# rhymes-ai/Aria

Measured on NVIDIA H100. Metric: Aria-25.3B bf16 prefill tokens/sec, higher is better.
Workload: dtype bf16

## Files before the change

aria_b200/csrc/gemm.cu:

```cuda
#include "gemm_common.cuh"

namespace aria {

constexpr int GEMM_STAGES = 4;
constexpr int acc_ld(int BN) { return BN + 4; }
template <int BN>
constexpr int gemm_smem_bytes() {
  return 1024  + GEMM_STAGES * (A_STAGE_BYTES + BN * BK * 2) + BM * acc_ld(BN) * 4 + 256 ;
}

template <int BN, bool B_MN>
ARIA_DEVICE void wgmma_tile_k16(float (&acc)[BN / 2], uint64_t da, uint64_t db) {
  if constexpr (BN == 128) wgmma_m64n128_ss<0, B_MN ? 1 : 0>(acc, da, db, 1u);
  else wgmma_m64n144_ss<0, B_MN ? 1 : 0>(acc, da, db, 1u);
}

template <int BN, bool B_MN, int EPI>
__global__ void __launch_bounds__(GEMM_THREADS, 1)
gemm_kernel(const __grid_constant__ CUtensorMap tmA, const __grid_constant__ CUtensorMap tmB0,
            const __grid_constant__ CUtensorMap tmB1, const __grid_constant__ CUtensorMap tmB2, const GemmParams p) {
  constexpr int B_STAGE_BYTES = BN * BK * 2;
  constexpr int STAGE_BYTES = A_STAGE_BYTES + B_STAGE_BYTES;
  constexpr int STAGES = GEMM_STAGES;
  constexpr int ACC_LD = acc_ld(BN);
  constexpr int OUT_BN = (EPI == ARIA_EPI_SWIGLU) ? BN / 2 : BN;
  static_assert(BN == 128 || BN == 144, "tile widths with a wgmma wrapper");

  extern __shared__ uint8_t smem_raw[];
  uint8_t* smem = reinterpret_cast<uint8_t*>((reinterpret_cast<uintptr_t>(smem_raw) + 1023) & ~uintptr_t(1023));
  float* stg = reinterpret_cast<float*>(smem + STAGES * STAGE_BYTES);
  uint64_t* full_bar = reinterpret_cast<uint64_t*>(stg + BM * ACC_LD);
  uint64_t* empty_bar = full_bar + STAGES;

  const int warp = threadIdx.x >> 5;
  const int lane = threadIdx.x & 31;
  const int wg = threadIdx.x >> 7;

  if (warp == 0 && lane == 0) {
    prefetch_tmap(&tmA);
    prefetch_tmap(&tmB0);
    if (p.n_seg > 1 || EPI == ARIA_EPI_SWIGLU) prefetch_tmap(&tmB1);
    if (p.n_seg > 2) prefetch_tmap(&tmB2);
    for (int i = 0; i < STAGES; ++i) {
      mbar_init(&full_bar[i], 1);
      mbar_init(&empty_bar[i], CONSUMER_WARPS);
    }
    fence_mbar_init();
  }
  __syncthreads();

  const int n_out_total = p.N * (EPI == ARIA_EPI_SWIGLU ? 1 : p.n_seg);
  const int n_tiles = (n_out_total + OUT_BN - 1) / OUT_BN;
  const int k_blocks = (p.K + BK - 1) / BK;
  const uint32_t smem_base = smem_u32(smem);
  const uint32_t full0 = smem_u32(full_bar), empty0 = smem_u32(empty_bar);

  if (wg == 0) {
    setmaxnreg_dec<40>();
    if (warp == 0 && elect_one()) {
      TileSched sched;
      sched.init(p, n_tiles);
      uint32_t stage = 0, phase = 0;
      for (int t = blockIdx.x;; t += gridDim.x) {
        int grp, m_idx, n_idx, row0, rows;
        if (!sched.decode(t, grp, m_idx, n_idx, row0, rows)) break;
        const int a_row = row0 + m_idx * BM;
        const int bgrp = weight_block(p, grp);
        int b_c0 = 0, b_c1 = 0;
        const CUtensorMap* tb0 = &tmB0;
        const CUtensorMap* tb1 = &tmB1;
        if constexpr (B_MN) {
          b_c0 = bgrp * p.K;
        } else if constexpr (EPI == ARIA_EPI_SWIGLU) {
          b_c0 = b_c1 = n_idx * OUT_BN;
        } else {
          const int col = n_idx * BN;
          const int seg = col / p.N;
          tb0 = seg == 0 ? &tmB0 : (seg == 1 ? &tmB1 : &tmB2);
          b_c0 = col - seg * p.N + bgrp * p.b_group_rows;
        }
        for (int kb = 0; kb < k_blocks; ++kb) {
          const uint32_t fb = full0 + stage * 8;
          const uint32_t sa = smem_base + stage * STAGE_BYTES;
          const uint32_t sb = sa + A_STAGE_BYTES;
          mbar_wait_addr(empty0 + stage * 8, phase ^ 1);
          mbar_arrive_expect_tx_addr(fb, STAGE_BYTES);
          tma_load_2d_addr(sa, &tmA, fb, kb * BK, a_row);
          if constexpr (B_MN) {
            const int krow = b_c0 + kb * BK;
            constexpr int CH = BN / 64;
#pragma unroll
            for (int c = 0; c < CH; ++c) {
              int ncol;
              if constexpr (EPI == ARIA_EPI_SWIGLU) {
                constexpr int HALF = CH / 2;
                ncol = (c < HALF) ? (n_idx * OUT_BN + c * 64) : (p.N + n_idx * OUT_BN + (c - HALF) * 64);
              } else {
                ncol = n_idx * BN + c * 64;
              }
              tma_load_2d_addr(sb + c * (64 * BK * 2), &tmB0, fb, ncol, krow);
            }
          } else if constexpr (EPI == ARIA_EPI_SWIGLU) {
            tma_load_2d_addr(sb, tb0, fb, kb * BK, b_c0);
            tma_load_2d_addr(sb + (BN / 2) * BK * 2, tb1, fb, kb * BK, b_c1);
          } else {
            tma_load_2d_addr(sb, tb0, fb, kb * BK, b_c0);
          }
          if (++stage == STAGES) {
            stage = 0;
            phase ^= 1;
          }
        }
      }
    }
  } else {
    setmaxnreg_inc<232>();
    const int cw = wg - 1;
    const int tid = threadIdx.x & 127;
    const uint32_t b_lbo = p.dbg_lbo ? p.dbg_lbo : (B_MN ? 64 * BK * 2 : 16);
    const uint32_t b_sbo = p.dbg_sbo ? p.dbg_sbo : 1024;
    const uint32_t b_kadv = (p.dbg_kadv ? p.dbg_kadv : (B_MN ? 16 * 128 : 32)) >> 4;
    const uint64_t da0 = make_smem_desc(smem_base + cw * 64 * 128, 16, 1024);
    const uint64_t db0 = make_smem_desc(smem_base + A_STAGE_BYTES, b_lbo, b_sbo);
    const int frag_row = cw * 64 + (tid >> 5) * 16 + (lane >> 2), frag_col = 2 * (lane & 3);
    const int epi_row = cw * 64 + (tid & 63), half = tid >> 6;
    TileSched sched;
    sched.init(p, n_tiles);
    uint32_t stage = 0, phase = 0;
    for (int t = blockIdx.x;; t += gridDim.x) {
      int grp, m_idx, n_idx, row0, rows;
      if (!sched.decode(t, grp, m_idx, n_idx, row0, rows)) break;
      float acc[BN / 2];
#pragma unroll
      for (int i = 0; i < BN / 2; ++i) acc[i] = 0.f;
      int prev = -1;
      for (int kb = 0; kb < k_blocks; ++kb) {
        mbar_wait_addr(full0 + stage * 8, phase);
        const uint64_t da = da0 + stage * (STAGE_BYTES >> 4);
        const uint64_t db = db0 + stage * (STAGE_BYTES >> 4);
        wgmma_fence();
#pragma unroll
        for (int k = 0; k < BK / 16; ++k) wgmma_tile_k16<BN, B_MN>(acc, da + k * 2, db + k * b_kadv);
        wgmma_commit();
        wgmma_wait<1>();
        if (prev >= 0 && lane == 0) mbar_arrive(&empty_bar[prev]);
        prev = static_cast<int>(stage);
        if (++stage == STAGES) {
          stage = 0;
          phase ^= 1;
        }
      }
      wgmma_wait<0>();
      fence_regs(acc);
      if (prev >= 0 && lane == 0) mbar_arrive(&empty_bar[prev]);

      named_bar_sync(1 + cw, 128);
#pragma unroll
      for (int j = 0; j < BN / 8; ++j) {
        float* d0 = stg + frag_row * ACC_LD + 8 * j + frag_col;
        *reinterpret_cast<float2*>(d0) = make_float2(acc[4 * j], acc[4 * j + 1]);
        *reinterpret_cast<float2*>(d0 + 8 * ACC_LD) = make_float2(acc[4 * j + 2], acc[4 * j + 3]);
      }
      named_bar_sync(1 + cw, 128);
      const int r_in_grp = m_idx * BM + epi_row;
      const bool row_ok = r_in_grp < rows;
      const int64_t grow = static_cast<int64_t>(row0) + r_in_grp;
      epilogue_tile<BN, EPI>(p, stg + epi_row * ACC_LD, n_out_total, n_idx, grow, row_ok, half, grp, r_in_grp);
    }
  }
}

template <int BN, bool B_MN, int EPI>
static int launch_gemm(const CUtensorMap& tmA, const CUtensorMap* tmB, const GemmParams& p, int max_tiles,
                       cudaStream_t stream) {
  constexpr int SMEM = gemm_smem_bytes<BN>();
  auto kern = gemm_kernel<BN, B_MN, EPI>;
  static bool attr_set[kMaxDevices] = {};
  if (ensure_dynamic_smem(attr_set, kern, SMEM) != cudaSuccess) return ARIA_ERR_CUDA;
  int grid = sm_count();
  if (max_tiles < grid) grid = max_tiles;
  if (grid < 1) grid = 1;
  kern<<<grid, GEMM_THREADS, SMEM, stream>>>(tmA, tmB[0], tmB[1], tmB[2], p);
  return check_launch("gemm_kernel");
}

}

using namespace aria;

extern "C" int aria_gemm(const aria_gemm_desc_t* d, aria_stream_t stream_) {
  cudaStream_t stream = reinterpret_cast<cudaStream_t>(stream_);
  ARIA_CHECK_ARG(d != nullptr);
  ARIA_CHECK_ARG(d->a && d->b[0] && d->out[0]);
  ARIA_CHECK_ARG(d->m >= 0 && d->n > 0 && d->k > 0);
  ARIA_CHECK_ARG(d->n % 8 == 0 && d->k % 8 == 0 && d->lda % 8 == 0);
  ARIA_CHECK_ARG(d->n_seg >= 1 && d->n_seg <= 3);
  ARIA_CHECK_ARG(d->num_groups >= 1 && (d->group_mod >= 0 || d->num_groups % (-d->group_mod) == 0));
  ARIA_CHECK_ARG((reinterpret_cast<uintptr_t>(d->a) & 15) == 0 && (reinterpret_cast<uintptr_t>(d->out[0]) & 15) == 0);
  if (d->m == 0) return ARIA_OK;
  const bool b_mn = d->b_layout == ARIA_B_GKN;
  const bool b_gnk = d->b_layout == ARIA_B_GNK;
  const bool swiglu = d->epilogue == ARIA_EPI_SWIGLU;
  if (b_mn) {
    ARIA_CHECK_ARG(d->n_seg == 1);
    ARIA_CHECK_ARG(d->k % BK == 0 || (d->num_groups == 1 && d->group_mod == 0));
    ARIA_CHECK_ARG(d->n % 64 == 0);
// ... 23 lines not shown
  p.n_seg = swiglu ? 1 : d->n_seg;
  p.act = d->act;
  for (int i = 0; i < 3; ++i) {
    p.bias[i] = static_cast<const __nv_bfloat16*>(d->bias[i]);
    p.out[i] = static_cast<__nv_bfloat16*>(d->out[i]);
  }
  p.residual = static_cast<const __nv_bfloat16*>(d->residual);
  p.ldr = d->ldr;
  p.ldo = d->ldo;
  p.head_dim = d->head_dim;
  p.head_ld = d->head_ld;
  p.rows_per_batch = d->rows_per_batch > 0 ? d->rows_per_batch : static_cast<int>(d->m);
  p.pos0 = d->pos0;
  p.stride_b = d->stride_b;
  p.stride_h = d->stride_h;
  p.rope_mask = d->rope_mask;
  p.rope_cos = static_cast<const __nv_bfloat16*>(d->rope_cos);
  p.rope_sin = static_cast<const __nv_bfloat16*>(d->rope_sin);
  p.position_ids = d->position_ids;
  p.dbg_lbo = d->dbg_lbo;
  p.dbg_sbo = d->dbg_sbo;
  p.dbg_kadv = d->dbg_kadv;

  const int64_t n_out_total = d->n * (swiglu ? 1 : d->n_seg);
  int BN = 128;
  if (d->epilogue == ARIA_EPI_HEADS) {
    ARIA_CHECK_ARG(d->head_dim > 0 && d->head_dim % 8 == 0 && d->head_ld >= d->head_dim && d->n % d->head_dim == 0);
    if (d->rope_mask) ARIA_CHECK_ARG(d->head_dim == 128 && d->rope_cos && d->rope_sin);
    if (d->n % 128 != 0) {
      ARIA_CHECK_ARG(!d->rope_mask && d->n % 144 == 0);
      BN = 144;
    }
    for (int s = 0; s < d->n_seg; ++s) ARIA_CHECK_ARG(d->out[s] && d->b[s]);
  } else {
    if (swiglu) ARIA_CHECK_ARG(d->n % 64 == 0);
    if (d->n_seg > 1 && !swiglu) ARIA_CHECK_ARG(d->n % BN == 0);
  }

  CUtensorMap tmA, tmB[3];
  int rc = make_tmap_2d(&tmA, d->a, d->k, d->a_rows > 0 ? d->a_rows : d->m, d->lda * 2, BK, BM);
  if (rc) return rc;
  if (b_mn) {
    const uint64_t ncols = swiglu ? 2 * d->n : d->n;
    const uint64_t n_weights = d->group_mod > 0 ? d->group_mod : (d->group_mod < 0 ? d->num_groups / (-d->group_mod) : d->num_groups);
    rc = make_tmap_2d(&tmB[0], d->b[0], ncols, n_weights * d->k, ncols * 2, 64, BK);
    if (rc) return rc;
    tmB[1] = tmB[0];
    tmB[2] = tmB[0];
  } else {
    const int nb = swiglu ? 2 : d->n_seg;
    const uint32_t box_rows = swiglu ? BN / 2 : BN;
    for (int s = 0; s < 3; ++s) {
      const void* ptr = s < nb ? d->b[s] : d->b[0];
      const uint64_t b_rows = b_gnk ? static_cast<uint64_t>(d->group_mod > 0 ? d->group_mod : (d->group_mod < 0 ? d->num_groups / (-d->group_mod) : d->num_groups)) * d->n : d->n;
      rc = make_tmap_2d(&tmB[s], ptr, d->k, b_rows, d->k * 2, BK, box_rows);
      if (rc) return rc;
    }
  }

  const int out_bn = swiglu ? BN / 2 : BN;
  const int64_t n_tiles = (n_out_total + out_bn - 1) / out_bn;
  const int64_t m_tiles_ub = (d->m + BM - 1) / BM + (d->num_groups > 1 ? d->num_groups : 0);
  int64_t max_tiles = n_tiles * m_tiles_ub;
  if (max_tiles > (1 << 30)) max_tiles = 1 << 30;

#define ARIA_LAUNCH(BN_, MN_, EPI_) return launch_gemm<BN_, MN_, EPI_>(tmA, tmB, p, static_cast<int>(max_tiles), stream)
  if (d->epilogue == ARIA_EPI_HEADS) {
    if (BN == 128) ARIA_LAUNCH(128, false, ARIA_EPI_HEADS);
    ARIA_LAUNCH(144, false, ARIA_EPI_HEADS);
  }
  if (swiglu) {
    if (b_mn) ARIA_LAUNCH(128, true, ARIA_EPI_SWIGLU);
    ARIA_LAUNCH(128, false, ARIA_EPI_SWIGLU);
  }
  if (b_mn) ARIA_LAUNCH(128, true, ARIA_EPI_LINEAR);
  ARIA_LAUNCH(128, false, ARIA_EPI_LINEAR);
#undef ARIA_LAUNCH
}

extern "C" int aria_grouped_gemm(const void* a, const void* b, void* out, const int32_t* group_offsets, int64_t rows,
                                 int64_t k, int64_t n, int32_t num_groups, aria_stream_t stream) {
  aria_gemm_desc_t d{};
  d.a = a;
  d.lda = k;
  d.m = rows;
  d.n = n;
  d.k = k;
  d.b[0] = b;
  d.n_seg = 1;
  d.b_layout = ARIA_B_GKN;
  d.num_groups = num_groups;
  d.group_offsets = group_offsets;
  d.epilogue = ARIA_EPI_LINEAR;
// ... 8 lines not shown
```

aria_b200/csrc/gemm_common.cuh:

```cuda
#pragma once
#include "common.cuh"
#include "ptx.cuh"

namespace aria {

constexpr int BM = 128;
constexpr int BK = 64;
constexpr int A_STAGE_BYTES = BM * BK * 2;
constexpr int GEMM_THREADS = 384;
constexpr int CONSUMER_WARPS = 8;

struct GemmParams {
  int M, N, K;
  int num_groups;
  const int32_t* group_offsets;
  const int32_t* group_counts;
  const uint64_t* out_group_base;
  const int32_t* out_group_row0;
  int b_group_rows;
  int group_mod;
  int n_seg;
  int act;
  const __nv_bfloat16* bias[3];
  const __nv_bfloat16* residual;
// ... 28 lines not shown
    g = -1;
    mt_prefix = 0;
    g_mt = 0;
    g_row0 = 0;
    g_rows = 0;
  }
  __device__ bool load_group(int gi) {
    if (gi >= G) return false;
    if (offs) {
      g_row0 = offs[gi];
      g_rows = cnts ? cnts[gi] : offs[gi + 1] - g_row0;
    } else {
      g_row0 = 0;
      g_rows = M;
    }
    g_mt = (g_rows + bm - 1) / bm;
    return true;
  }
  __device__ bool decode(int t, int& grp, int& m_idx, int& n_idx, int& row0, int& rows) {
    if (g < 0) {
      g = 0;
      if (!load_group(0)) return false;
    }
    while (t >= (mt_prefix + g_mt) * n_tiles) {
      mt_prefix += g_mt;
      ++g;
      if (!load_group(g)) return false;
    }
    int r = t - mt_prefix * n_tiles;
    n_idx = r / g_mt;
    m_idx = r - n_idx * g_mt;
    grp = g;
    row0 = g_row0;
    rows = g_rows;
    return true;
  }
};

ARIA_DEVICE float act_apply(float x, int act) {
  if (act == ARIA_ACT_GELU_TANH) {
    const float k0 = 0.7978845608028654f, k1 = 0.044715f;
    float inner = k0 * (x + k1 * x * x * x);
    return 0.5f * x * (1.f + fast_tanh(inner));
  }
  if (act == ARIA_ACT_GELU_NEW) {
    float p3 = bf16r(x * x * x);
    float t = bf16r(0.044715f * p3);
    t = bf16r(x + t);
    t = bf16r(0.7978845608028654f * t);
    t = bf16r(fast_tanh(t));
    t = bf16r(1.0f + t);
    float h = bf16r(0.5f * x);
    return h * t;
  }
  return x;
}

ARIA_DEVICE void ld_acc32(const float* src, uint32_t (&r)[32]) {
#pragma unroll
  for (int i = 0; i < 8; ++i) {
    const uint4 v = *reinterpret_cast<const uint4*>(src + 4 * i);
    r[4 * i] = v.x;
    r[4 * i + 1] = v.y;
    r[4 * i + 2] = v.z;
    r[4 * i + 3] = v.w;
  }
}

template <int BN, int EPI>
ARIA_DEVICE void epilogue_tile(const GemmParams& p, const float* acc, const int n_out_total, const int n_idx,
                               const int64_t grow, const bool row_ok, const int half, const int grp = 0, const int r_in_grp = 0) {
  constexpr int OUT_BN = (EPI == ARIA_EPI_SWIGLU) ? BN / 2 : BN;
  if constexpr (EPI == ARIA_EPI_SWIGLU) {
    __nv_bfloat16* orow = p.out[0] + grow * p.ldo + n_idx * OUT_BN;
    constexpr int NCH = OUT_BN / 32;
    const int cb = (half * NCH / 2) * 32, ce = half ? OUT_BN : (NCH / 2) * 32;
#pragma unroll 1
    for (int c = cb; c < ce; c += 32) {
      uint32_t g[32], u[32];
      ld_acc32(acc + c, g);
      ld_acc32(acc + OUT_BN + c, u);
      uint32_t o[16];
#pragma unroll
      for (int j = 0; j < 32; j += 2) {
        float g0 = __uint_as_float(g[j]), g1 = __uint_as_float(g[j + 1]);
        float u0 = __uint_as_float(u[j]), u1 = __uint_as_float(u[j + 1]);
        bf16r2(g0, g1);
        bf16r2(u0, u1);
        float s0 = fast_silu(g0), s1 = fast_silu(g1);
        bf16r2(s0, s1);
        o[j >> 1] = pack_bf16(s0 * u0, s1 * u1);
      }
      if (row_ok) {
#pragma unroll
        for (int q = 0; q < 4; ++q) {
          const int col = n_idx * OUT_BN + c + q * 8;
          if (col + 8 <= p.N)
            *reinterpret_cast<uint4*>(orow + c + q * 8) = make_uint4(o[q * 4], o[q * 4 + 1], o[q * 4 + 2], o[q * 4 + 3]);
        }
      }
    }
  } else if constexpr (EPI == ARIA_EPI_LINEAR) {
    const int col0 = n_idx * BN;
    const int seg = col0 / p.N;
    const __nv_bfloat16* bias = p.bias[seg];
    __nv_bfloat16* orow = p.out[0] + grow * p.ldo + col0;
    if (p.out_group_base)
      orow = reinterpret_cast<__nv_bfloat16*>(p.out_group_base[grp]) + static_cast<int64_t>(p.out_group_row0[grp] + r_in_grp) * p.ldo + col0;
    const __nv_bfloat16* rrow = (p.residual && row_ok) ? p.residual + grow * p.ldr + col0 : nullptr;
    constexpr int NCH = BN / 32, NCHH = NCH - NCH / 2;
    const int cb = half ? (NCH / 2) * 32 : 0;
    const int n_my = half ? NCH - NCH / 2 : NCH / 2;
    if (n_my == 0) return;
    uint32_t v[2][32];
    uint4 bv[2][4], rv[2][4];
    auto issue = [&](int c, int set) {
      ld_acc32(acc + c, v[set]);
#pragma unroll
      for (int q = 0; q < 4; ++q) {
        const int col = col0 + c + q * 8;
        const bool ok = col + 8 <= n_out_total;
        bv[set][q] = (bias && ok) ? __ldg(reinterpret_cast<const uint4*>(bias + (col - seg * p.N))) : make_uint4(0, 0, 0, 0);
        rv[set][q] = (rrow && ok) ? *reinterpret_cast<const uint4*>(rrow + c + q * 8) : make_uint4(0, 0, 0, 0);
      }
    };
    issue(cb, 0);
#pragma unroll
    for (int i = 0; i < NCHH; ++i) {
      if (i >= n_my) break;
      const int c = cb + i * 32;
      const int set = i & 1;
      if (i + 1 < n_my) issue(c + 32, set ^ 1);
#pragma unroll
      for (int q = 0; q < 4; ++q) {
        const int col = col0 + c + q * 8;
        if (col + 8 > n_out_total) continue;
        float x[8];
#pragma unroll
        for (int j = 0; j < 8; ++j) x[j] = __uint_as_float(v[set][q * 8 + j]);
        if (bias) {
          const uint32_t bw[4] = {bv[set][q].x, bv[set][q].y, bv[set][q].z, bv[set][q].w};
#pragma unroll
          for (int j = 0; j < 4; ++j) {
            x[2 * j] += bf16_lo(bw[j]);
            x[2 * j + 1] += bf16_hi(bw[j]);
          }
        }
#pragma unroll
        for (int j = 0; j < 8; ++j) x[j] = bf16r(x[j]);
        if (p.act != ARIA_ACT_NONE) {
#pragma unroll
          for (int j = 0; j < 8; ++j) x[j] = bf16r(act_apply(x[j], p.act));
        }
        if (row_ok) {
          if (rrow) {
            const uint32_t rw[4] = {rv[set][q].x, rv[set][q].y, rv[set][q].z, rv[set][q].w};
#pragma unroll
            for (int j = 0; j < 4; ++j) {
              x[2 * j] += bf16_lo(rw[j]);
              x[2 * j + 1] += bf16_hi(rw[j]);
            }
          }
          *reinterpret_cast<uint4*>(orow + c + q * 8) =
              make_uint4(pack_bf16(x[0], x[1]), pack_bf16(x[2], x[3]), pack_bf16(x[4], x[5]), pack_bf16(x[6], x[7]));
        }
      }
    }
  } else {
    const int col0 = n_idx * BN;
    const int seg = col0 / p.N;
    const int cseg0 = col0 - seg * p.N;
    const __nv_bfloat16* bias = p.bias[seg];
    const int b = static_cast<int>(grow / p.rows_per_batch);
    const int tok = static_cast<int>(grow - static_cast<int64_t>(b) * p.rows_per_batch);
    __nv_bfloat16* obase = p.out[seg] + b * p.stride_b + static_cast<int64_t>(p.pos0 + tok) * p.head_ld;
    const bool rope = (p.rope_mask >> seg) & 1;
    if (rope) {
      const int pos = row_ok ? (p.position_ids ? p.position_ids[grow] : p.pos0 + tok) : 0;
      const __nv_bfloat16* cs = p.rope_cos + static_cast<int64_t>(pos) * p.head_dim;
      const __nv_bfloat16* sn = p.rope_sin + static_cast<int64_t>(pos) * p.head_dim;
      constexpr int NHC = BN / 64;
#pragma unroll 1
      for (int hc = half * NHC / 2; hc < (half ? NHC : NHC / 2); hc += 1) {
        const int hh = hc >> 1, c = (hc & 1) * 32;
        __nv_bfloat16* orow = obase + (cseg0 / p.head_dim + hh) * p.stride_h;
        const float* th = acc + hh * 128;
        uint32_t lo[32], hi[32];
        ld_acc32(th + c, lo);
        ld_acc32(th + 64 + c, hi);
        uint4 tc_lo[4], ts_lo[4], tc_hi[4], ts_hi[4];
#pragma unroll
        for (int q = 0; q < 4; ++q) {
          tc_lo[q] = __ldg(reinterpret_cast<const uint4*>(cs + c + q * 8));
          ts_lo[q] = __ldg(reinterpret_cast<const uint4*>(sn + c + q * 8));
          tc_hi[q] = __ldg(reinterpret_cast<const uint4*>(cs + 64 + c + q * 8));
          ts_hi[q] = __ldg(reinterpret_cast<const uint4*>(sn + 64 + c + q * 8));
        }
        if (row_ok) {
#pragma unroll
          for (int q = 0; q < 4; ++q) {
            const uint4 c_lo = tc_lo[q], s_lo = ts_lo[q], c_hi = tc_hi[q], s_hi = ts_hi[q];
            const uint32_t cl[4] = {c_lo.x, c_lo.y, c_lo.z, c_lo.w}, sl[4] = {s_lo.x, s_lo.y, s_lo.z, s_lo.w};
            const uint32_t ch[4] = {c_hi.x, c_hi.y, c_hi.z, c_hi.w}, sh[4] = {s_hi.x, s_hi.y, s_hi.z, s_hi.w};
            float ol[8], oh[8];
#pragma unroll
            for (int j = 0; j < 8; ++j) {
              float xl = __uint_as_float(lo[q * 8 + j]);
              float xh = __uint_as_float(hi[q * 8 + j]);
              bf16r2(xl, xh);
              float cosl = (j & 1) ? bf16_hi(cl[j >> 1]) : bf16_lo(cl[j >> 1]);
              float sinl = (j & 1) ? bf16_hi(sl[j >> 1]) : bf16_lo(sl[j >> 1]);
              float cosh_ = (j & 1) ? bf16_hi(ch[j >> 1]) : bf16_lo(ch[j >> 1]);
              float sinh_ = (j & 1) ? bf16_hi(sh[j >> 1]) : bf16_lo(sh[j >> 1]);
              float a0 = xl * cosl, a1 = -xh * sinl, b0 = xh * cosh_, b1 = xl * sinh_;
              bf16r2(a0, a1);
              bf16r2(b0, b1);
              ol[j] = a0 + a1;
              oh[j] = b0 + b1;
            }
            *reinterpret_cast<uint4*>(orow + c + q * 8) =
                make_uint4(pack_bf16(ol[0], ol[1]), pack_bf16(ol[2], ol[3]), pack_bf16(ol[4], ol[5]), pack_bf16(ol[6], ol[7]));
            *reinterpret_cast<uint4*>(orow + 64 + c + q * 8) =
                make_uint4(pack_bf16(oh[0], oh[1]), pack_bf16(oh[2], oh[3]), pack_bf16(oh[4], oh[5]), pack_bf16(oh[6], oh[7]));
          }
        }
      }
    } else {
      constexpr int NCH = (BN + 31) / 32, NMAX = NCH - NCH / 2;
      const int cb = half ? (NCH / 2) * 32 : 0;
      const int n_my = half ? NCH - NCH / 2 : NCH / 2;
      uint32_t v[2][32];
      uint4 bvq[2][4];
      auto window = [&](int c) { return (c + 32 <= BN) ? c : BN - 32; };
      auto issue = [&](int c, int set) {
        const int cbase = window(c);
        ld_acc32(acc + cbase, v[set]);
#pragma unroll
        for (int q = 0; q < 4; ++q) {
          const int cs_ = cseg0 + cbase + q * 8;
          bvq[set][q] = (bias && cs_ + 8 <= p.N) ? __ldg(reinterpret_cast<const uint4*>(bias + cs_)) : make_uint4(0, 0, 0, 0);
        }
      };
      if (n_my > 0) issue(cb, 0);
#pragma unroll
      for (int i = 0; i < NMAX; ++i) {
        if (i >= n_my) break;
        const int c = cb + i * 32;
        const int set = i & 1;
        if (i + 1 < n_my) issue(c + 32, set ^ 1);
        const int cbase = window(c);
        const int qstart = (c + 32 <= BN) ? 0 : (c - cbase) / 8;
#pragma unroll
        for (int q = 0; q < 4; ++q) {
          if (q < qstart) continue;
          const int cs_ = cseg0 + cbase + q * 8;
          if (cs_ + 8 > p.N) continue;
          float x[8];
#pragma unroll
          for (int j = 0; j < 8; ++j) x[j] = __uint_as_float(v[set][q * 8 + j]);
          if (bias) {
            const uint4 bv = bvq[set][q];
            const uint32_t bw[4] = {bv.x, bv.y, bv.z, bv.w};
#pragma unroll
            for (int j = 0; j < 4; ++j) {
              x[2 * j] += bf16_lo(bw[j]);
              x[2 * j + 1] += bf16_hi(bw[j]);
            }
          }
          if (row_ok) {
            const int head = cs_ / p.head_dim;
            const int d = cs_ - head * p.head_dim;
            *reinterpret_cast<uint4*>(obase + head * p.stride_h + d) =
                make_uint4(pack_bf16(x[0], x[1]), pack_bf16(x[2], x[3]), pack_bf16(x[4], x[5]), pack_bf16(x[6], x[7]));
          }
        }
      }
    }
  }
}

}
```

aria_b200/csrc/ptx.cuh:

```cuda
#pragma once
#include <cuda.h>
#include <cuda_bf16.h>
#include <cuda_runtime.h>
#include <stdint.h>

namespace aria {

#define ARIA_DEVICE __device__ __forceinline__

ARIA_DEVICE uint32_t smem_u32(const void* p) { return static_cast<uint32_t>(__cvta_generic_to_shared(p)); }

ARIA_DEVICE uint32_t elect_one() {
  uint32_t pred = 0;
  asm volatile(
      "{\n\t.reg .pred P;\n\t"
      "elect.sync _|P, 0xffffffff;\n\t"
      "selp.b32 %0, 1, 0, P;\n\t}\n"
      : "=r"(pred));
  return pred;
}

ARIA_DEVICE void mbar_init(uint64_t* bar, uint32_t count) {
  asm volatile("mbarrier.init.shared::cta.b64 [%0], %1;" ::"r"(smem_u32(bar)), "r"(count));
}
// ... 89 lines not shown
template <int R> ARIA_DEVICE void fence_regs(float (&d)[R]) {
#pragma unroll
  for (int i = 0; i < R; ++i) asm volatile("" : "+f"(d[i])::"memory");
}
ARIA_DEVICE void named_bar_sync(uint32_t id, uint32_t threads) { asm volatile("bar.sync %0, %1;" ::"r"(id), "r"(threads) : "memory"); }
ARIA_DEVICE void named_bar_arrive(uint32_t id, uint32_t threads) { asm volatile("bar.arrive %0, %1;" ::"r"(id), "r"(threads) : "memory"); }

template <int TA, int TB>
ARIA_DEVICE void wgmma_m64n128_ss(float (&d)[64], uint64_t da, uint64_t db, uint32_t scale_d) {
  asm volatile(
      "{\n\t.reg .pred p;\n\tsetp.ne.b32 p, %66, 0;\n\t"
      "wgmma.mma_async.sync.aligned.m64n128k16.f32.bf16.bf16 {%0, %1, %2, %3, %4, %5, %6, %7, %8, %9, %10, %11, %12, %13, %14, %15, %16, %17, %18, %19, %20, %21, %22, %23, %24, %25, %26, %27, %28, %29, %30, %31, %32, %33, %34, %35, %36, %37, %38, %39, %40, %41, %42, %43, %44, %45, %46, %47, %48, %49, %50, %51, %52, %53, %54, %55, %56, %57, %58, %59, %60, %61, %62, %63}, %64, %65, p, 1, 1, %67, %68;\n\t}\n"
      : "+f"(d[0]), "+f"(d[1]), "+f"(d[2]), "+f"(d[3]), "+f"(d[4]), "+f"(d[5]), "+f"(d[6]), "+f"(d[7]), "+f"(d[8]), "+f"(d[9]), "+f"(d[10]), "+f"(d[11]), "+f"(d[12]), "+f"(d[13]), "+f"(d[14]), "+f"(d[15]), "+f"(d[16]), "+f"(d[17]), "+f"(d[18]), "+f"(d[19]), "+f"(d[20]), "+f"(d[21]), "+f"(d[22]), "+f"(d[23]), "+f"(d[24]), "+f"(d[25]), "+f"(d[26]), "+f"(d[27]), "+f"(d[28]), "+f"(d[29]), "+f"(d[30]), "+f"(d[31]), "+f"(d[32]), "+f"(d[33]), "+f"(d[34]), "+f"(d[35]), "+f"(d[36]), "+f"(d[37]), "+f"(d[38]), "+f"(d[39]), "+f"(d[40]), "+f"(d[41]), "+f"(d[42]), "+f"(d[43]), "+f"(d[44]), "+f"(d[45]), "+f"(d[46]), "+f"(d[47]), "+f"(d[48]), "+f"(d[49]), "+f"(d[50]), "+f"(d[51]), "+f"(d[52]), "+f"(d[53]), "+f"(d[54]), "+f"(d[55]), "+f"(d[56]), "+f"(d[57]), "+f"(d[58]), "+f"(d[59]), "+f"(d[60]), "+f"(d[61]), "+f"(d[62]), "+f"(d[63])
      : "l"(da), "l"(db), "r"(scale_d), "n"(TA), "n"(TB));
}
template <int TA, int TB>
ARIA_DEVICE void wgmma_m64n64_ss(float (&d)[32], uint64_t da, uint64_t db, uint32_t scale_d) {
  asm volatile(
      "{\n\t.reg .pred p;\n\tsetp.ne.b32 p, %34, 0;\n\t"
      "wgmma.mma_async.sync.aligned.m64n64k16.f32.bf16.bf16 {%0, %1, %2, %3, %4, %5, %6, %7, %8, %9, %10, %11, %12, %13, %14, %15, %16, %17, %18, %19, %20, %21, %22, %23, %24, %25, %26, %27, %28, %29, %30, %31}, %32, %33, p, 1, 1, %35, %36;\n\t}\n"
      : "+f"(d[0]), "+f"(d[1]), "+f"(d[2]), "+f"(d[3]), "+f"(d[4]), "+f"(d[5]), "+f"(d[6]), "+f"(d[7]), "+f"(d[8]), "+f"(d[9]), "+f"(d[10]), "+f"(d[11]), "+f"(d[12]), "+f"(d[13]), "+f"(d[14]), "+f"(d[15]), "+f"(d[16]), "+f"(d[17]), "+f"(d[18]), "+f"(d[19]), "+f"(d[20]), "+f"(d[21]), "+f"(d[22]), "+f"(d[23]), "+f"(d[24]), "+f"(d[25]), "+f"(d[26]), "+f"(d[27]), "+f"(d[28]), "+f"(d[29]), "+f"(d[30]), "+f"(d[31])
      : "l"(da), "l"(db), "r"(scale_d), "n"(TA), "n"(TB));
}
template <int TA, int TB>
ARIA_DEVICE void wgmma_m64n144_ss(float (&d)[72], uint64_t da, uint64_t db, uint32_t scale_d) {
  asm volatile(
      "{\n\t.reg .pred p;\n\tsetp.ne.b32 p, %74, 0;\n\t"
      "wgmma.mma_async.sync.aligned.m64n144k16.f32.bf16.bf16 {%0, %1, %2, %3, %4, %5, %6, %7, %8, %9, %10, %11, %12, %13, %14, %15, %16, %17, %18, %19, %20, %21, %22, %23, %24, %25, %26, %27, %28, %29, %30, %31, %32, %33, %34, %35, %36, %37, %38, %39, %40, %41, %42, %43, %44, %45, %46, %47, %48, %49, %50, %51, %52, %53, %54, %55, %56, %57, %58, %59, %60, %61, %62, %63, %64, %65, %66, %67, %68, %69, %70, %71}, %72, %73, p, 1, 1, %75, %76;\n\t}\n"
      : "+f"(d[0]), "+f"(d[1]), "+f"(d[2]), "+f"(d[3]), "+f"(d[4]), "+f"(d[5]), "+f"(d[6]), "+f"(d[7]), "+f"(d[8]), "+f"(d[9]), "+f"(d[10]), "+f"(d[11]), "+f"(d[12]), "+f"(d[13]), "+f"(d[14]), "+f"(d[15]), "+f"(d[16]), "+f"(d[17]), "+f"(d[18]), "+f"(d[19]), "+f"(d[20]), "+f"(d[21]), "+f"(d[22]), "+f"(d[23]), "+f"(d[24]), "+f"(d[25]), "+f"(d[26]), "+f"(d[27]), "+f"(d[28]), "+f"(d[29]), "+f"(d[30]), "+f"(d[31]), "+f"(d[32]), "+f"(d[33]), "+f"(d[34]), "+f"(d[35]), "+f"(d[36]), "+f"(d[37]), "+f"(d[38]), "+f"(d[39]), "+f"(d[40]), "+f"(d[41]), "+f"(d[42]), "+f"(d[43]), "+f"(d[44]), "+f"(d[45]), "+f"(d[46]), "+f"(d[47]), "+f"(d[48]), "+f"(d[49]), "+f"(d[50]), "+f"(d[51]), "+f"(d[52]), "+f"(d[53]), "+f"(d[54]), "+f"(d[55]), "+f"(d[56]), "+f"(d[57]), "+f"(d[58]), "+f"(d[59]), "+f"(d[60]), "+f"(d[61]), "+f"(d[62]), "+f"(d[63]), "+f"(d[64]), "+f"(d[65]), "+f"(d[66]), "+f"(d[67]), "+f"(d[68]), "+f"(d[69]), "+f"(d[70]), "+f"(d[71])
      : "l"(da), "l"(db), "r"(scale_d), "n"(TA), "n"(TB));
}
template <int TB>
ARIA_DEVICE void wgmma_m64n128_rs(float (&d)[64], const uint32_t (&a)[4], uint64_t db) {
  asm volatile(
      "{\n\t.reg .pred p;\n\tsetp.ne.b32 p, 1, 0;\n\t"
      "wgmma.mma_async.sync.aligned.m64n128k16.f32.bf16.bf16 {%0, %1, %2, %3, %4, %5, %6, %7, %8, %9, %10, %11, %12, %13, %14, %15, %16, %17, %18, %19, %20, %21, %22, %23, %24, %25, %26, %27, %28, %29, %30, %31, %32, %33, %34, %35, %36, %37, %38, %39, %40, %41, %42, %43, %44, %45, %46, %47, %48, %49, %50, %51, %52, %53, %54, %55, %56, %57, %58, %59, %60, %61, %62, %63}, {%64, %65, %66, %67}, %68, p, 1, 1, %69;\n\t}\n"
      : "+f"(d[0]), "+f"(d[1]), "+f"(d[2]), "+f"(d[3]), "+f"(d[4]), "+f"(d[5]), "+f"(d[6]), "+f"(d[7]), "+f"(d[8]), "+f"(d[9]), "+f"(d[10]), "+f"(d[11]), "+f"(d[12]), "+f"(d[13]), "+f"(d[14]), "+f"(d[15]), "+f"(d[16]), "+f"(d[17]), "+f"(d[18]), "+f"(d[19]), "+f"(d[20]), "+f"(d[21]), "+f"(d[22]), "+f"(d[23]), "+f"(d[24]), "+f"(d[25]), "+f"(d[26]), "+f"(d[27]), "+f"(d[28]), "+f"(d[29]), "+f"(d[30]), "+f"(d[31]), "+f"(d[32]), "+f"(d[33]), "+f"(d[34]), "+f"(d[35]), "+f"(d[36]), "+f"(d[37]), "+f"(d[38]), "+f"(d[39]), "+f"(d[40]), "+f"(d[41]), "+f"(d[42]), "+f"(d[43]), "+f"(d[44]), "+f"(d[45]), "+f"(d[46]), "+f"(d[47]), "+f"(d[48]), "+f"(d[49]), "+f"(d[50]), "+f"(d[51]), "+f"(d[52]), "+f"(d[53]), "+f"(d[54]), "+f"(d[55]), "+f"(d[56]), "+f"(d[57]), "+f"(d[58]), "+f"(d[59]), "+f"(d[60]), "+f"(d[61]), "+f"(d[62]), "+f"(d[63])
      : "r"(a[0]), "r"(a[1]), "r"(a[2]), "r"(a[3]), "l"(db), "n"(TB));
}
template <int TB>
ARIA_DEVICE void wgmma_m64n64_rs(float (&d)[32], const uint32_t (&a)[4], uint64_t db) {
  asm volatile(
      "{\n\t.reg .pred p;\n\tsetp.ne.b32 p, 1, 0;\n\t"
      "wgmma.mma_async.sync.aligned.m64n64k16.f32.bf16.bf16 {%0, %1, %2, %3, %4, %5, %6, %7, %8, %9, %10, %11, %12, %13, %14, %15, %16, %17, %18, %19, %20, %21, %22, %23, %24, %25, %26, %27, %28, %29, %30, %31}, {%32, %33, %34, %35}, %36, p, 1, 1, %37;\n\t}\n"
      : "+f"(d[0]), "+f"(d[1]), "+f"(d[2]), "+f"(d[3]), "+f"(d[4]), "+f"(d[5]), "+f"(d[6]), "+f"(d[7]), "+f"(d[8]), "+f"(d[9]), "+f"(d[10]), "+f"(d[11]), "+f"(d[12]), "+f"(d[13]), "+f"(d[14]), "+f"(d[15]), "+f"(d[16]), "+f"(d[17]), "+f"(d[18]), "+f"(d[19]), "+f"(d[20]), "+f"(d[21]), "+f"(d[22]), "+f"(d[23]), "+f"(d[24]), "+f"(d[25]), "+f"(d[26]), "+f"(d[27]), "+f"(d[28]), "+f"(d[29]), "+f"(d[30]), "+f"(d[31])
      : "r"(a[0]), "r"(a[1]), "r"(a[2]), "r"(a[3]), "l"(db), "n"(TB));
}
template <int TB>
ARIA_DEVICE void wgmma_m64n16_rs(float (&d)[8], const uint32_t (&a)[4], uint64_t db) {
  asm volatile(
      "{\n\t.reg .pred p;\n\tsetp.ne.b32 p, 1, 0;\n\t"
      "wgmma.mma_async.sync.aligned.m64n16k16.f32.bf16.bf16 {%0, %1, %2, %3, %4, %5, %6, %7}, {%8, %9, %10, %11}, %12, p, 1, 1, %13;\n\t}\n"
      : "+f"(d[0]), "+f"(d[1]), "+f"(d[2]), "+f"(d[3]), "+f"(d[4]), "+f"(d[5]), "+f"(d[6]), "+f"(d[7])
      : "r"(a[0]), "r"(a[1]), "r"(a[2]), "r"(a[3]), "l"(db), "n"(TB));
// ... 37 lines not shown
```

Before: 16570.

## Add ping-pong consumer schedule to GEMM and drop 144-wide tiles

Adds a ping-pong mode in which the two consumer warpgroups each own a full 128-row tile and alternate, coordinated by named barriers, so one group's epilogue overlaps the other's MMA main loop. The mode is chosen when there are at least two tiles per CTA and no activation. It also removes the 144-column tile path and reworks tile indexing per segment. The heads epilogue now packs results to shared memory and copies them out in a separate coalesced pass. The trade-offs are more barrier synchronisation, a shared staging buffer, and 128-wide tiles for head dims that previously used 144.

```diff
diff --git a/aria_b200/csrc/gemm.cu b/aria_b200/csrc/gemm.cu
--- a/aria_b200/csrc/gemm.cu
+++ b/aria_b200/csrc/gemm.cu
@@ -9,13 +9,9 @@
   return 1024  + GEMM_STAGES * (A_STAGE_BYTES + BN * BK * 2) + BM * acc_ld(BN) * 4 + 256 ;
 }
 
-template <int BN, bool B_MN>
-ARIA_DEVICE void wgmma_tile_k16(float (&acc)[BN / 2], uint64_t da, uint64_t db) {
-  if constexpr (BN == 128) wgmma_m64n128_ss<0, B_MN ? 1 : 0>(acc, da, db, 1u);
-  else wgmma_m64n144_ss<0, B_MN ? 1 : 0>(acc, da, db, 1u);
-}
-
-template <int BN, bool B_MN, int EPI>
+constexpr uint32_t BAR_STG = 1, BAR_TURN = 3, BAR_FREE = 5;
+
+template <int BN, bool B_MN, int EPI, bool PP>
 __global__ void __launch_bounds__(GEMM_THREADS, 1)
 gemm_kernel(const __grid_constant__ CUtensorMap tmA, const __grid_constant__ CUtensorMap tmB0,
             const __grid_constant__ CUtensorMap tmB1, const __grid_constant__ CUtensorMap tmB2, const GemmParams p) {
@@ -24,7 +20,8 @@
   constexpr int STAGES = GEMM_STAGES;
   constexpr int ACC_LD = acc_ld(BN);
   constexpr int OUT_BN = (EPI == ARIA_EPI_SWIGLU) ? BN / 2 : BN;
-  static_assert(BN == 128 || BN == 144, "tile widths with a wgmma wrapper");
+  static_assert(BN == 128, "tile width of the wgmma wrapper");
+  static_assert((STAGES & (STAGES - 1)) == 0, "ring positions map to stages by masking");
 
   extern __shared__ uint8_t smem_raw[];
   uint8_t* smem = reinterpret_cast<uint8_t*>((reinterpret_cast<uintptr_t>(smem_raw) + 1023) & ~uintptr_t(1023));
@@ -43,14 +40,15 @@
     if (p.n_seg > 2) prefetch_tmap(&tmB2);
     for (int i = 0; i < STAGES; ++i) {
       mbar_init(&full_bar[i], 1);
-      mbar_init(&empty_bar[i], CONSUMER_WARPS);
+      mbar_init(&empty_bar[i], PP ? CONSUMER_WARPS / 2 : CONSUMER_WARPS);
     }
     fence_mbar_init();
   }
   __syncthreads();
 
   const int n_out_total = p.N * (EPI == ARIA_EPI_SWIGLU ? 1 : p.n_seg);
-  const int n_tiles = (n_out_total + OUT_BN - 1) / OUT_BN;
+  const int n_tiles_seg = (p.N + OUT_BN - 1) / OUT_BN;
+  const int n_tiles = n_tiles_seg * p.n_seg;
   const int k_blocks = (p.K + BK - 1) / BK;
   const uint32_t smem_base = smem_u32(smem);
   const uint32_t full0 = smem_u32(full_bar), empty0 = smem_u32(empty_bar);
@@ -74,10 +72,9 @@
         } else if constexpr (EPI == ARIA_EPI_SWIGLU) {
           b_c0 = b_c1 = n_idx * OUT_BN;
         } else {
-          const int col = n_idx * BN;
-          const int seg = col / p.N;
+          const int seg = n_idx / n_tiles_seg;
           tb0 = seg == 0 ? &tmB0 : (seg == 1 ? &tmB1 : &tmB2);
-          b_c0 = col - seg * p.N + bgrp * p.b_group_rows;
+          b_c0 = (n_idx - seg * n_tiles_seg) * BN + bgrp * p.b_group_rows;
         }
         for (int kb = 0; kb < k_blocks; ++kb) {
           const uint32_t fb = full0 + stage * 8;
@@ -113,6 +110,76 @@
         }
       }
     }
+  } else if constexpr (PP) {
+    setmaxnreg_inc<232>();
+    const int cw = wg - 1;
+    const int tid = threadIdx.x & 127;
+    const uint32_t b_lbo = p.dbg_lbo ? p.dbg_lbo : (B_MN ? 64 * BK * 2 : 16);
+    const uint32_t b_sbo = p.dbg_sbo ? p.dbg_sbo : 1024;
+    const uint32_t b_kadv = (p.dbg_kadv ? p.dbg_kadv : (B_MN ? 16 * 128 : 32)) >> 4;
+    const uint64_t da0 = make_smem_desc(smem_base, 16, 1024);
+    const uint64_t db0 = make_smem_desc(smem_base + A_STAGE_BYTES, b_lbo, b_sbo);
+    constexpr uint64_t DA_HI = (64 * 128) >> 4;
+    const int frag_row = (tid >> 5) * 16 + (lane >> 2), frag_col = 2 * (lane & 3);
+    const uint32_t other = cw ^ 1;
+    TileSched sched;
+    sched.init(p, n_tiles);
+    int grp, m_idx, n_idx, row0, rows;
+    if (cw == 1 && sched.decode(blockIdx.x, grp, m_idx, n_idx, row0, rows)) {
+      named_bar_arrive(BAR_TURN + 0, 256);
+      named_bar_arrive(BAR_FREE + 0, 256);
+    }
+    uint32_t pos = cw * k_blocks;
+    for (int t = blockIdx.x + cw * gridDim.x;; t += 2 * gridDim.x) {
+      if (!sched.decode(t, grp, m_idx, n_idx, row0, rows)) break;
+      int g2, m2, n2, r2, c2;
+      const bool other_next = sched.decode(t + gridDim.x, g2, m2, n2, r2, c2);
+      float acc0[BN / 2], acc1[BN / 2];
+#pragma unroll
+      for (int i = 0; i < BN / 2; ++i) acc0[i] = acc1[i] = 0.f;
+      named_bar_sync(BAR_TURN + cw, 256);
+      int prev = -1;
+      for (int kb = 0; kb < k_blocks; ++kb, ++pos) {
+        const uint32_t stage = pos & (STAGES - 1);
+        mbar_wait_addr(full0 + stage * 8, (pos / STAGES) & 1);
+        const uint64_t da = da0 + stage * (STAGE_BYTES >> 4);
+        const uint64_t db = db0 + stage * (STAGE_BYTES >> 4);
+        wgmma_fence();
+#pragma unroll
+        for (int k = 0; k < BK / 16; ++k) {
+          wgmma_m64n128_ss<0, B_MN ? 1 : 0>(acc0, da + k * 2, db + k * b_kadv, 1u);
+          wgmma_m64n128_ss<0, B_MN ? 1 : 0>(acc1, da + DA_HI + k * 2, db + k * b_kadv, 1u);
+        }
+        wgmma_commit();
+        if (kb == k_blocks - 1 && other_next) named_bar_arrive(BAR_TURN + other, 256);
+        wgmma_wait<1>();
+        if (prev >= 0 && lane == 0) mbar_arrive(&empty_bar[prev]);
+        prev = static_cast<int>(stage);
+      }
+      wgmma_wait<0>();
+      fence_regs(acc0);
+      fence_regs(acc1);
+      if (prev >= 0 && lane == 0) mbar_arrive(&empty_bar[prev]);
+      pos += k_blocks;
+
+      named_bar_sync(BAR_FREE + cw, 256);
+#pragma unroll
+      for (int j = 0; j < BN / 8; ++j) {
+        float* d0 = stg + frag_row * ACC_LD + 8 * j + frag_col;
+        *reinterpret_cast<float2*>(d0) = make_float2(acc0[4 * j], acc0[4 * j + 1]);
+        *reinterpret_cast<float2*>(d0 + 8 * ACC_LD) = make_float2(acc0[4 * j + 2], acc0[4 * j + 3]);
+        *reinterpret_cast<float2*>(d0 + 64 * ACC_LD) = make_float2(acc1[4 * j], acc1[4 * j + 1]);
+        *reinterpret_cast<float2*>(d0 + 72 * ACC_LD) = make_float2(acc1[4 * j + 2], acc1[4 * j + 3]);
+      }
+      named_bar_sync(BAR_STG + cw, 128);
+      const int r_in_grp = m_idx * BM + tid;
+      const bool row_ok = r_in_grp < rows;
+      epilogue_tile<BN, EPI, 1>(p, stg + tid * ACC_LD, n_out_total, n_tiles_seg, n_idx, row0 + r_in_grp, row_ok, 0, grp,
+                                r_in_grp);
+      if constexpr (EPI == ARIA_EPI_HEADS)
+        heads_copy_out<BN, 1, BM>(p, stg, ACC_LD, 0, tid, BAR_STG + cw, n_tiles_seg, n_idx, m_idx, row0, rows);
+      if (other_next) named_bar_arrive(BAR_FREE + other, 256);
+    }
   } else {
     setmaxnreg_inc<232>();
     const int cw = wg - 1;
@@ -140,7 +207,7 @@
         const uint64_t db = db0 + stage * (STAGE_BYTES >> 4);
         wgmma_fence();
 #pragma unroll
-        for (int k = 0; k < BK / 16; ++k) wgmma_tile_k16<BN, B_MN>(acc, da + k * 2, db + k * b_kadv);
+        for (int k = 0; k < BK / 16; ++k) wgmma_m64n128_ss<0, B_MN ? 1 : 0>(acc, da + k * 2, db + k * b_kadv, 1u);
         wgmma_commit();
         wgmma_wait<1>();
         if (prev >= 0 && lane == 0) mbar_arrive(&empty_bar[prev]);
@@ -154,34 +221,42 @@
       fence_regs(acc);
       if (prev >= 0 && lane == 0) mbar_arrive(&empty_bar[prev]);
 
-      named_bar_sync(1 + cw, 128);
+      named_bar_sync(BAR_STG + cw, 128);
 #pragma unroll
       for (int j = 0; j < BN / 8; ++j) {
         float* d0 = stg + frag_row * ACC_LD + 8 * j + frag_col;
         *reinterpret_cast<float2*>(d0) = make_float2(acc[4 * j], acc[4 * j + 1]);
         *reinterpret_cast<float2*>(d0 + 8 * ACC_LD) = make_float2(acc[4 * j + 2], acc[4 * j + 3]);
       }
-      named_bar_sync(1 + cw, 128);
+      named_bar_sync(BAR_STG + cw, 128);
       const int r_in_grp = m_idx * BM + epi_row;
       const bool row_ok = r_in_grp < rows;
-      const int64_t grow = static_cast<int64_t>(row0) + r_in_grp;
-      epilogue_tile<BN, EPI>(p, stg + epi_row * ACC_LD, n_out_total, n_idx, grow, row_ok, half, grp, r_in_grp);
-    }
-  }
+      epilogue_tile<BN, EPI, 2>(p, stg + epi_row * ACC_LD, n_out_total, n_tiles_seg, n_idx, row0 + r_in_grp, row_ok, half, grp,
+                                r_in_grp);
+      if constexpr (EPI == ARIA_EPI_HEADS)
+        heads_copy_out<BN, 2, 64>(p, stg, ACC_LD, cw * 64, tid, BAR_STG + cw, n_tiles_seg, n_idx, m_idx, row0, rows);
+    }
+  }
+}
+
+template <int BN, bool B_MN, int EPI, bool PP>
+static int launch_gemm_as(const CUtensorMap& tmA, const CUtensorMap* tmB, const GemmParams& p, int grid, cudaStream_t stream) {
+  constexpr int SMEM = gemm_smem_bytes<BN>();
+  auto kern = gemm_kernel<BN, B_MN, EPI, PP>;
+  static bool attr_set[kMaxDevices] = {};
+  if (ensure_dynamic_smem(attr_set, kern, SMEM) != cudaSuccess) return ARIA_ERR_CUDA;
+  kern<<<grid, GEMM_THREADS, SMEM, stream>>>(tmA, tmB[0], tmB[1], tmB[2], p);
+  return check_launch("gemm_kernel");
 }
 
 template <int BN, bool B_MN, int EPI>
 static int launch_gemm(const CUtensorMap& tmA, const CUtensorMap* tmB, const GemmParams& p, int max_tiles,
                        cudaStream_t stream) {
-  constexpr int SMEM = gemm_smem_bytes<BN>();
-  auto kern = gemm_kernel<BN, B_MN, EPI>;
-  static bool attr_set[kMaxDevices] = {};
-  if (ensure_dynamic_smem(attr_set, kern, SMEM) != cudaSuccess) return ARIA_ERR_CUDA;
   int grid = sm_count();
   if (max_tiles < grid) grid = max_tiles;
   if (grid < 1) grid = 1;
-  kern<<<grid, GEMM_THREADS, SMEM, stream>>>(tmA, tmB[0], tmB[1], tmB[2], p);
-  return check_launch("gemm_kernel");
+  if (max_tiles >= 2 * grid && p.act == ARIA_ACT_NONE) return launch_gemm_as<BN, B_MN, EPI, true>(tmA, tmB, p, grid, stream);
+  return launch_gemm_as<BN, B_MN, EPI, false>(tmA, tmB, p, grid, stream);
 }
 
 }
@@ -251,15 +326,10 @@
   p.dbg_sbo = d->dbg_sbo;
   p.dbg_kadv = d->dbg_kadv;
 
-  const int64_t n_out_total = d->n * (swiglu ? 1 : d->n_seg);
-  int BN = 128;
+  constexpr int BN = 128;
   if (d->epilogue == ARIA_EPI_HEADS) {
     ARIA_CHECK_ARG(d->head_dim > 0 && d->head_dim % 8 == 0 && d->head_ld >= d->head_dim && d->n % d->head_dim == 0);
     if (d->rope_mask) ARIA_CHECK_ARG(d->head_dim == 128 && d->rope_cos && d->rope_sin);
-    if (d->n % 128 != 0) {
-      ARIA_CHECK_ARG(!d->rope_mask && d->n % 144 == 0);
-      BN = 144;
-    }
     for (int s = 0; s < d->n_seg; ++s) ARIA_CHECK_ARG(d->out[s] && d->b[s]);
   } else {
     if (swiglu) ARIA_CHECK_ARG(d->n % 64 == 0);
@@ -288,16 +358,13 @@
   }
 
   const int out_bn = swiglu ? BN / 2 : BN;
-  const int64_t n_tiles = (n_out_total + out_bn - 1) / out_bn;
+  const int64_t n_tiles = (d->n + out_bn - 1) / out_bn * p.n_seg;
   const int64_t m_tiles_ub = (d->m + BM - 1) / BM + (d->num_groups > 1 ? d->num_groups : 0);
   int64_t max_tiles = n_tiles * m_tiles_ub;
   if (max_tiles > (1 << 30)) max_tiles = 1 << 30;
 
 #define ARIA_LAUNCH(BN_, MN_, EPI_) return launch_gemm<BN_, MN_, EPI_>(tmA, tmB, p, static_cast<int>(max_tiles), stream)
-  if (d->epilogue == ARIA_EPI_HEADS) {
-    if (BN == 128) ARIA_LAUNCH(128, false, ARIA_EPI_HEADS);
-    ARIA_LAUNCH(144, false, ARIA_EPI_HEADS);
-  }
+  if (d->epilogue == ARIA_EPI_HEADS) ARIA_LAUNCH(128, false, ARIA_EPI_HEADS);
   if (swiglu) {
     if (b_mn) ARIA_LAUNCH(128, true, ARIA_EPI_SWIGLU);
     ARIA_LAUNCH(128, false, ARIA_EPI_SWIGLU);
diff --git a/aria_b200/csrc/gemm_common.cuh b/aria_b200/csrc/gemm_common.cuh
--- a/aria_b200/csrc/gemm_common.cuh
+++ b/aria_b200/csrc/gemm_common.cuh
@@ -74,6 +74,7 @@
       g = 0;
       if (!load_group(0)) return false;
     }
+    if (g >= G) return false;
     while (t >= (mt_prefix + g_mt) * n_tiles) {
       mt_prefix += g_mt;
       ++g;
@@ -119,16 +120,16 @@
   }
 }
 
-template <int BN, int EPI>
-ARIA_DEVICE void epilogue_tile(const GemmParams& p, const float* acc, const int n_out_total, const int n_idx,
-                               const int64_t grow, const bool row_ok, const int half, const int grp = 0, const int r_in_grp = 0) {
+template <int BN, int EPI, int PARTS>
+ARIA_DEVICE void epilogue_tile(const GemmParams& p, float* acc, const int n_out_total, const int n_tiles_seg,
+                               const int n_idx, const int grow, const bool row_ok, const int part, const int grp = 0,
+                               const int r_in_grp = 0) {
   constexpr int OUT_BN = (EPI == ARIA_EPI_SWIGLU) ? BN / 2 : BN;
   if constexpr (EPI == ARIA_EPI_SWIGLU) {
     __nv_bfloat16* orow = p.out[0] + grow * p.ldo + n_idx * OUT_BN;
-    constexpr int NCH = OUT_BN / 32;
-    const int cb = (half * NCH / 2) * 32, ce = half ? OUT_BN : (NCH / 2) * 32;
+    constexpr int NCP = OUT_BN / 32 / PARTS;
 #pragma unroll 1
-    for (int c = cb; c < ce; c += 32) {
+    for (int c = part * NCP * 32; c < (part + 1) * NCP * 32; c += 32) {
       uint32_t g[32], u[32];
       ld_acc32(acc + c, g);
       ld_acc32(acc + OUT_BN + c, u);
@@ -160,10 +161,8 @@
     if (p.out_group_base)
       orow = reinterpret_cast<__nv_bfloat16*>(p.out_group_base[grp]) + static_cast<int64_t>(p.out_group_row0[grp] + r_in_grp) * p.ldo + col0;
     const __nv_bfloat16* rrow = (p.residual && row_ok) ? p.residual + grow * p.ldr + col0 : nullptr;
-    constexpr int NCH = BN / 32, NCHH = NCH - NCH / 2;
-    const int cb = half ? (NCH / 2) * 32 : 0;
-    const int n_my = half ? NCH - NCH / 2 : NCH / 2;
-    if (n_my == 0) return;
+    constexpr int NCP = BN / 32 / PARTS;
+    const int cb = part * NCP * 32;
     uint32_t v[2][32];
     uint4 bv[2][4], rv[2][4];
     auto issue = [&](int c, int set) {
@@ -178,11 +177,10 @@
     };
     issue(cb, 0);
 #pragma unroll
-    for (int i = 0; i < NCHH; ++i) {
-      if (i >= n_my) break;
+    for (int i = 0; i < NCP; ++i) {
       const int c = cb + i * 32;
       const int set = i & 1;
-      if (i + 1 < n_my) issue(c + 32, set ^ 1);
+      if (i + 1 < NCP) issue(c + 32, set ^ 1);
 #pragma unroll
       for (int q = 0; q < 4; ++q) {
         const int col = col0 + c + q * 8;
@@ -219,21 +217,20 @@
       }
     }
   } else {
-    const int col0 = n_idx * BN;
-    const int seg = col0 / p.N;
-    const int cseg0 = col0 - seg * p.N;
+    const int seg = n_idx / n_tiles_seg;
+    const int cseg0 = (n_idx - seg * n_tiles_seg) * BN;
     const __nv_bfloat16* bias = p.bias[seg];
-    const int b = static_cast<int>(grow / p.rows_per_batch);
-    const int tok = static_cast<int>(grow - static_cast<int64_t>(b) * p.rows_per_batch);
-    __nv_bfloat16* obase = p.out[seg] + b * p.stride_b + static_cast<int64_t>(p.pos0 + tok) * p.head_ld;
     const bool rope = (p.rope_mask >> seg) & 1;
     if (rope) {
+      const int b = grow / p.rows_per_batch;
+      const int tok = grow - b * p.rows_per_batch;
+      __nv_bfloat16* obase = p.out[seg] + b * p.stride_b + static_cast<int64_t>(p.pos0 + tok) * p.head_ld;
       const int pos = row_ok ? (p.position_ids ? p.position_ids[grow] : p.pos0 + tok) : 0;
       const __nv_bfloat16* cs = p.rope_cos + static_cast<int64_t>(pos) * p.head_dim;
       const __nv_bfloat16* sn = p.rope_sin + static_cast<int64_t>(pos) * p.head_dim;
-      constexpr int NHC = BN / 64;
+      constexpr int NHCP = BN / 64 / PARTS;
 #pragma unroll 1
-      for (int hc = half * NHC / 2; hc < (half ? NHC : NHC / 2); hc += 1) {
+      for (int hc = part * NHCP; hc < (part + 1) * NHCP; hc += 1) {
         const int hh = hc >> 1, c = (hc & 1) * 32;
         __nv_bfloat16* orow = obase + (cseg0 / p.head_dim + hh) * p.stride_h;
         const float* th = acc + hh * 128;
@@ -278,34 +275,27 @@
         }
       }
     } else {
-      constexpr int NCH = (BN + 31) / 32, NMAX = NCH - NCH / 2;
-      const int cb = half ? (NCH / 2) * 32 : 0;
-      const int n_my = half ? NCH - NCH / 2 : NCH / 2;
+      constexpr int NCP = BN / 32 / PARTS;
+      const int cb = part * NCP * 32;
       uint32_t v[2][32];
       uint4 bvq[2][4];
-      auto window = [&](int c) { return (c + 32 <= BN) ? c : BN - 32; };
       auto issue = [&](int c, int set) {
-        const int cbase = window(c);
-        ld_acc32(acc + cbase, v[set]);
+        ld_acc32(acc + c, v[set]);
 #pragma unroll
         for (int q = 0; q < 4; ++q) {
-          const int cs_ = cseg0 + cbase + q * 8;
+          const int cs_ = cseg0 + c + q * 8;
           bvq[set][q] = (bias && cs_ + 8 <= p.N) ? __ldg(reinterpret_cast<const uint4*>(bias + cs_)) : make_uint4(0, 0, 0, 0);
         }
       };
-      if (n_my > 0) issue(cb, 0);
-#pragma unroll
-      for (int i = 0; i < NMAX; ++i) {
-        if (i >= n_my) break;
+      issue(cb, 0);
+#pragma unroll
+      for (int i = 0; i < NCP; ++i) {
         const int c = cb + i * 32;
         const int set = i & 1;
-        if (i + 1 < n_my) issue(c + 32, set ^ 1);
-        const int cbase = window(c);
-        const int qstart = (c + 32 <= BN) ? 0 : (c - cbase) / 8;
+        if (i + 1 < NCP) issue(c + 32, set ^ 1);
 #pragma unroll
         for (int q = 0; q < 4; ++q) {
-          if (q < qstart) continue;
-          const int cs_ = cseg0 + cbase + q * 8;
+          const int cs_ = cseg0 + c + q * 8;
           if (cs_ + 8 > p.N) continue;
           float x[8];
 #pragma unroll
@@ -319,16 +309,40 @@
               x[2 * j + 1] += bf16_hi(bw[j]);
             }
           }
-          if (row_ok) {
-            const int head = cs_ / p.head_dim;
-            const int d = cs_ - head * p.head_dim;
-            *reinterpret_cast<uint4*>(obase + head * p.stride_h + d) =
-                make_uint4(pack_bf16(x[0], x[1]), pack_bf16(x[2], x[3]), pack_bf16(x[4], x[5]), pack_bf16(x[6], x[7]));
-          }
-        }
-      }
-    }
-  }
-}
-
-}
+          *reinterpret_cast<uint4*>(reinterpret_cast<char*>(acc) + 4 * cb + 2 * (c + q * 8 - cb)) =
+              make_uint4(pack_bf16(x[0], x[1]), pack_bf16(x[2], x[3]), pack_bf16(x[4], x[5]), pack_bf16(x[6], x[7]));
+        }
+      }
+    }
+  }
+}
+
+template <int BN, int PARTS, int NROWS>
+ARIA_DEVICE void heads_copy_out(const GemmParams& p, const float* stg, const int acc_ld, const int row_begin, const int tid,
+                                const uint32_t bar, const int n_tiles_seg, const int n_idx, const int m_idx, const int row0,
+                                const int rows) {
+  const int seg = n_idx / n_tiles_seg;
+  if ((p.rope_mask >> seg) & 1) return;
+  const int cseg0 = (n_idx - seg * n_tiles_seg) * BN;
+  constexpr int PPR = BN / 8;
+  constexpr int PART_COLS = BN / PARTS;
+  named_bar_sync(bar, 128);
+#pragma unroll 4
+  for (int i = tid; i < NROWS * PPR; i += 128) {
+    const int r = row_begin + i / PPR, c = (i % PPR) * 8;
+    const int cs_ = cseg0 + c;
+    const int r_in_grp = m_idx * BM + r;
+    if (cs_ + 8 > p.N || r_in_grp >= rows) continue;
+    const int part = c / PART_COLS;
+    const uint4 v = *reinterpret_cast<const uint4*>(reinterpret_cast<const char*>(stg + r * acc_ld) + 4 * part * PART_COLS +
+                                                    2 * (c - part * PART_COLS));
+    const int grow = row0 + r_in_grp;
+    const int b = grow / p.rows_per_batch;
+    const int tok = grow - b * p.rows_per_batch;
+    const int head = cs_ / p.head_dim;
+    const int d = cs_ - head * p.head_dim;
+    *reinterpret_cast<uint4*>(p.out[seg] + b * p.stride_b + static_cast<int64_t>(p.pos0 + tok) * p.head_ld + head * p.stride_h + d) = v;
+  }
+}
+
+}
diff --git a/aria_b200/csrc/ptx.cuh b/aria_b200/csrc/ptx.cuh
--- a/aria_b200/csrc/ptx.cuh
+++ b/aria_b200/csrc/ptx.cuh
@@ -135,14 +135,6 @@
       : "+f"(d[0]), "+f"(d[1]), "+f"(d[2]), "+f"(d[3]), "+f"(d[4]), "+f"(d[5]), "+f"(d[6]), "+f"(d[7]), "+f"(d[8]), "+f"(d[9]), "+f"(d[10]), "+f"(d[11]), "+f"(d[12]), "+f"(d[13]), "+f"(d[14]), "+f"(d[15]), "+f"(d[16]), "+f"(d[17]), "+f"(d[18]), "+f"(d[19]), "+f"(d[20]), "+f"(d[21]), "+f"(d[22]), "+f"(d[23]), "+f"(d[24]), "+f"(d[25]), "+f"(d[26]), "+f"(d[27]), "+f"(d[28]), "+f"(d[29]), "+f"(d[30]), "+f"(d[31])
       : "l"(da), "l"(db), "r"(scale_d), "n"(TA), "n"(TB));
 }
-template <int TA, int TB>
-ARIA_DEVICE void wgmma_m64n144_ss(float (&d)[72], uint64_t da, uint64_t db, uint32_t scale_d) {
-  asm volatile(
-      "{\n\t.reg .pred p;\n\tsetp.ne.b32 p, %74, 0;\n\t"
-      "wgmma.mma_async.sync.aligned.m64n144k16.f32.bf16.bf16 {%0, %1, %2, %3, %4, %5, %6, %7, %8, %9, %10, %11, %12, %13, %14, %15, %16, %17, %18, %19, %20, %21, %22, %23, %24, %25, %26, %27, %28, %29, %30, %31, %32, %33, %34, %35, %36, %37, %38, %39, %40, %41, %42, %43, %44, %45, %46, %47, %48, %49, %50, %51, %52, %53, %54, %55, %56, %57, %58, %59, %60, %61, %62, %63, %64, %65, %66, %67, %68, %69, %70, %71}, %72, %73, p, 1, 1, %75, %76;\n\t}\n"
-      : "+f"(d[0]), "+f"(d[1]), "+f"(d[2]), "+f"(d[3]), "+f"(d[4]), "+f"(d[5]), "+f"(d[6]), "+f"(d[7]), "+f"(d[8]), "+f"(d[9]), "+f"(d[10]), "+f"(d[11]), "+f"(d[12]), "+f"(d[13]), "+f"(d[14]), "+f"(d[15]), "+f"(d[16]), "+f"(d[17]), "+f"(d[18]), "+f"(d[19]), "+f"(d[20]), "+f"(d[21]), "+f"(d[22]), "+f"(d[23]), "+f"(d[24]), "+f"(d[25]), "+f"(d[26]), "+f"(d[27]), "+f"(d[28]), "+f"(d[29]), "+f"(d[30]), "+f"(d[31]), "+f"(d[32]), "+f"(d[33]), "+f"(d[34]), "+f"(d[35]), "+f"(d[36]), "+f"(d[37]), "+f"(d[38]), "+f"(d[39]), "+f"(d[40]), "+f"(d[41]), "+f"(d[42]), "+f"(d[43]), "+f"(d[44]), "+f"(d[45]), "+f"(d[46]), "+f"(d[47]), "+f"(d[48]), "+f"(d[49]), "+f"(d[50]), "+f"(d[51]), "+f"(d[52]), "+f"(d[53]), "+f"(d[54]), "+f"(d[55]), "+f"(d[56]), "+f"(d[57]), "+f"(d[58]), "+f"(d[59]), "+f"(d[60]), "+f"(d[61]), "+f"(d[62]), "+f"(d[63]), "+f"(d[64]), "+f"(d[65]), "+f"(d[66]), "+f"(d[67]), "+f"(d[68]), "+f"(d[69]), "+f"(d[70]), "+f"(d[71])
-      : "l"(da), "l"(db), "r"(scale_d), "n"(TA), "n"(TB));
-}
 template <int TB>
 ARIA_DEVICE void wgmma_m64n128_rs(float (&d)[64], const uint32_t (&a)[4], uint64_t db) {
   asm volatile(
```

Measured after the change: 18240, median of 6. 10.1% higher.
